# Gavinli-lgf/belief-planning

Hardware: AMD Instinct MI355X
Metric: branch-MPC solves/sec (whole node), highway N=20 M=3 branches, batch 4096 egos (higher is better)
Workload: dtype f64; 1 GPU; highway BranchMPC_CVaR closed loop, N=20, NB=1, m=3 (T=64, U=61), 4096 egos per GPU; batch_per_gpu=4096, global_batch=4096, world_size=1, parallelism=ego-sharded dp1, loop=per step: k_env + solve launches

## Files before the change

### __graft_entry__.py

```python
import os
import sys

REPO = os.path.dirname(os.path.abspath(__file__))
PKG = os.path.join(REPO, "belief-planning_amd")
for _p in (REPO, PKG, os.path.join(REPO, "tests")):
    if _p not in sys.path:
        sys.path.insert(0, _p)


def build() -> None:
    from bmpc import _lib
    _lib.build(force=True, verbose=True)
    _lib.load()
    _lib.build_variant("rec0", ["-DBMPC_ITER_RECORD=0"])
    import hostsim_lib
    hostsim_lib.build()
    import bmpc.plan
    import MPC_branch
    import highway_branch_dyn
    print("build ok:", _lib.SO_PATH)


def smoke() -> None:
    import numpy as np
    from bmpc import plan
    from bmpc.scenarios import highway_desc, highway_policy_rows, seeded_batch
    from oracle.ecos_ipm import ecos_solve
    from oracle.model import HighwayModel, highway_policies
    from oracle.tree import CVaRController
# ... 36 lines not shown
```

### belief-planning_amd/csrc/bmpc_core.h

```cpp
#pragma once

#include <stddef.h>
#include <stdint.h>

#include "bmpc.h"

#ifndef BMPC_PHASE_NOCSR
#define BMPC_PHASE_NOCSR 1
#endif
#if BMPC_PHASE_NOCSR && defined(__HIP_DEVICE_COMPILE__)
#define BMPC_FN_CALLS __attribute__((not_tail_called))
#else
#define BMPC_FN_CALLS
#endif
#ifndef BMPC_ITER_RECORD
#define BMPC_ITER_RECORD 1
#endif
#define BMPC_ITER_LDS 32
#if defined(__HIPCC__)
#include <hip/hip_runtime.h>
#define BMPC_HD __host__ __device__ __forceinline__
#if defined(BMPC_INLINE_ALL)
#define BMPC_FN __host__ __device__ __forceinline__
#else
#define BMPC_FN __host__ __device__ __attribute__((noinline)) BMPC_FN_CALLS
#endif
#else
#define BMPC_HD inline
#define BMPC_FN inline
#endif

// ... 428 lines not shown
```

### belief-planning_amd/csrc/bmpc_ipm.h

```cpp
#pragma once

#include <type_traits>

#include "bmpc_tree.h"
#include "bmpc_wave.h"

#ifndef BMPC_EQUIL
#define BMPC_EQUIL 1
#endif
#ifndef BMPC_EQUIL_ITERS
#define BMPC_EQUIL_ITERS 3
#endif
#ifndef BMPC_TS_POST_RB_MIN
#define BMPC_TS_POST_RB_MIN 8
#endif
#ifndef BMPC_TS_POST_RB
#define BMPC_TS_POST_RB 4
#endif
#ifndef BMPC_PAIR_REFINE
#define BMPC_PAIR_REFINE 1
#endif
#ifndef BMPC_BLK_WAVE_SUBST
#define BMPC_BLK_WAVE_SUBST 1
#endif
// ... 537 lines not shown
  BMPC_TOC(C.ws, *C.L, PROF_G_CONE, t_gcone);
  ex.sync();
}
template <class X, int NX, int NU, int WM>
BMPC_FN_APPLY_G void apply_G_call(const X ex, const Ctx Cin, const gdouble* zv, gdouble* out, const gdouble* r3h,
                                  gdouble* tr) {
  apply_G_body<X, NX, NU, WM>(ex, Cin, zv, out, r3h, tr);
}
template <class X, int NX, int NU, int WM>
BMPC_HD void apply_G(const X ex, const Ctx& C, const gdouble* zv, gdouble* out, const gdouble* r3h, gdouble* tr) {
  if constexpr (inline_g<X>::value) apply_G_body<X, NX, NU, WM>(ex, C, zv, out, r3h, tr);
  else apply_G_call<X, NX, NU, WM>(ex, C, zv, out, r3h, tr);
}

template <class X, int NX, int NU>
BMPC_FN_APPLY_GT void apply_GT(const X ex, const Ctx Cin, const gdouble* r, gdouble* out, const gdouble* add = nullptr) {
  const Ctx C = Cin.uniform();
  add = uniform_ptr(add);
  const double sa = add ? 1.0 : 0.0;
  const gdouble* ad = add ? add : r;
  double qx[NX];
  ctx_qx<NX>(C, qx);
  CPlan& P = *C.P;
  BMPC_PROF(C.ws, *C.L, PROF_APPLYGT);
  const auto t = topo_view(P, ex);
  const int Nc = P.Nc;
  const gdouble* boost = C.at(C.L->boost);
  const gdouble* dh = C.at(C.L->dh);
  const double Qs = P.desc.Qslack[1];
  for (int k = ex.lane; k < P.T; k += ex.nlanes) {
    double ax[NX], cx[NX], os[BMPC_MAX_FX + 1];
#pragma unroll
    for (int j = 0; j < NX; ++j) ax[j] = 0.0, cx[j] = 0.0;
    const bool term = t.x_u[k] < 0;
    double fS = 0.0;
// ... 12 lines not shown
    } else if (k == 0) {
      const int kr = P.ncones - 1;
      const int off = t.cone_off[kr], q = t.cone_q[kr];
      fS = Qs * (r[off] - r[off + q - 1]) * ebeta<X>(boost, P.ncones, kr);
    }
    double dhk[NX];
#pragma unroll
    for (int j = 0; j < NX; ++j) dhk[j] = dh[k * NX + j];
    for (int c = 0; c < Nc; ++c) {
      const double rv = r[P.rFx + k * Nc + c];
      if (!term)
#pragma unroll
        for (int j = 0; j < NX; ++j) ax[j] += (c == 0 ? -dhk[j] : fxv(P, ex, c - 1, j)) * rv;
      os[c] = -rv - r[P.rPos + k * Nc + c] + fS;
    }
    for (int c = 0; c < Nc; ++c) out[P.oS + k * Nc + c] = os[c] + sa * ad[P.oS + k * Nc + c];
#pragma unroll
    for (int j = 0; j < NX; ++j) out[P.oX + k * NX + j] = (kc >= 0 ? ax[j] + cx[j] : ax[j]) + sa * ad[P.oX + k * NX + j];
  }
  for (int u = ex.lane; u < P.U; u += ex.nlanes) {
    double au[NU];
#pragma unroll
    for (int j = 0; j < NU; ++j) au[j] = 0.0;
    for (int rr = 0; rr < P.nFu; ++rr) {
      const double rv = r[P.rFu + u * P.nFu + rr];
#pragma unroll
      for (int j = 0; j < NU; ++j) au[j] += P.desc.Fu[rr * NU + j] * rv;
    }
    const int kc = t.u_cone[u];
    if (kc >= 0) {
      const int off = t.cone_off[kc];
      const int c = t.cone_c[kc];
      const int base = c >= 0 ? 1 + P.N * NX + (u - t.br_ndu[c]) * NU : 1;
#pragma unroll
      for (int s2 = 0; s2 < NU; ++s2) {
        double v = 0.0;
#pragma unroll
        for (int rr = 0; rr < NU; ++rr) v += -2.0 * P.Wu[rr * NU + s2] * r[off + base + rr];
        au[s2] += v;
      }
    }
#pragma unroll
    for (int j = 0; j < NU; ++j) out[P.oU + u * NU + j] = au[j] + sa * ad[P.oU + u * NU + j];
  }
  for (int i = ex.lane; i < P.ng; i += ex.nlanes) {
    double v = 0.0;
    const int gi = i == P.ng - 1 ? P.oJ : P.oRho + i;
    if (gi < P.oSig) v = -r[P.rRisk + (gi - P.oRho)];
    else if (gi >= P.oMup && gi < P.oS) v = -r[P.rRisk + P.bdim + (gi - P.oMup)];
    for (int k = 0; k < P.ncones; ++k) {
      const int off = t.cone_off[k], q = t.cone_q[k], c = t.cone_c[k];
      double w = 0.0;
      if (c >= 0) {
        const int b = t.cone_b[k], ii = t.cone_i[k];
        if (gi == P.oSig + b) w += 1.0;
        if (gi == P.oMup + b + ii) w += 1.0;
        if (gi == P.oMum + b + ii) w -= 1.0;
        if (t.br_child0[c] >= 0 && gi == P.oRho + c) w += 1.0;
      } else {
        if (gi == P.oJ) w -= 1.0;
        if (gi == P.oRho) w += 1.0;
      }
      if (w != 0.0) v += w * (r[off] - r[off + q - 1]) * ebeta<X>(boost, P.ncones, k);
    }
    out[gi] = v + sa * ad[gi];
  }
  ex.sync();
}

template <class X, int NX, int NU>
BMPC_HD void apply_A(const X ex, const Ctx& C, const gdouble* zv, gdouble* out) {
  CPlan& P = *C.P;
  const auto t = topo_view(P, ex);
  const gdouble* Ad = C.at(C.L->Ad);
  const gdouble* Bd = C.at(C.L->Bd);
  struct V4 { double v[NX]; };
  lane_batch<2>(ex, 0, P.T, [&](int k) {
    const int su = t.x_srcu[k], sx = t.x_srcx[k];
    V4 o;
#pragma unroll
    for (int r = 0; r < NX; ++r) o.v[r] = zv[P.oX + k * NX + r];
    if (su >= 0) {
      double xs[NX], us[NU];
// ... 408 lines not shown
#pragma unroll
    for (int uu = 0; uu < UC; ++uu) {
      const int i = G.gl + uu * G.cg;
      if (i < q) out1[off + i] = y[uu];
    }
    cone_W_regs<UC>(ex, G, a, y, cone_row0<UC>(ex, G, y), sc, v);
#pragma unroll
    for (int uu = 0; uu < UC; ++uu) {
      const int i = G.gl + uu * G.cg;
      if (i < q) out2[off + i] = v[uu];
    }
  }
  ex.sync();
}

template <class X>
BMPC_FN_FUSED LpSteps affine_dirs(const X ex, const Ctx Cin, const gdouble* z2, const gdouble* z1, double t,
                                  const gdouble* lam, gdouble* rb, gdouble* ds) {
  const Ctx C = Cin.uniform();
  z2 = uniform_ptr(z2), z1 = uniform_ptr(z1), lam = uniform_ptr(lam), rb = uniform_ptr(rb), ds = uniform_ptr(ds);
  CPlan& P = *C.P;
  LpSteps m{1e300, 1e300};
  if (!cone_regs(ex, P)) {
    gdouble* dz = C.at(C.L->dz);
    lane_batch<8>(ex, 0, P.nrows, [&](int i) { return z2[i] + t * z1[i]; }, [&](int i, double v) { dz[i] = v; });
    ex.sync();
    apply_W(ex, C, 0, dz, rb);
    lane_batch<8>(ex, 0, P.nrows, [&](int i) { return -lam[i] - rb[i]; }, [&](int i, double v) { ds[i] = v; });
    ex.sync();
    return BMPC_IPM_LEAN_PASSES ? lp_steps(ex, P, lam, ds, rb) : m;
// ... 104 lines not shown
        rb[off + i] = y[uu];
        ds[off + i] = d[uu];
      }
    }
    cone_W_regs<UC>(ex, G, a, d, cone_row0<UC>(ex, G, d), sc, v);
#pragma unroll
    for (int uu = 0; uu < UC; ++uu) {
      const int i = G.gl + uu * G.cg;
      if (i < q) rc[off + i] = v[uu];
    }
  }
  ex.sync();
  return m;
}

template <class X>
BMPC_FN_FUSED void combined_rhs(const X ex, const Ctx Cin, const gdouble* lam, gdouble* ds, gdouble* rb,
                                const gdouble* rz, double smu, double eta1) {
  const Ctx C = Cin.uniform();
  lam = uniform_ptr(lam), ds = uniform_ptr(ds), rb = uniform_ptr(rb), rz = uniform_ptr(rz);
  CPlan& P = *C.P;
  if (!cone_regs(ex, P)) {
    gdouble* ra = C.at(C.L->ra);
    gdouble* rc = C.at(C.L->rc);
    jprod(ex, C, lam, lam, ra);
    jprod(ex, C, ds, rb, rc);
    lane_batch<8>(ex, 0, P.nrows, [&](int i) {
      const double v = -ra[i] - rc[i];
      return i < P.nlp ? v + smu : v;
    }, [&](int i, double v) { ra[i] = v; });
    ex.sync();
    for (int k = ex.lane; k < P.ncones; k += ex.nlanes) ra[topo_view(P, ex).cone_off[k]] += smu;
    ex.sync();
    jdiv(ex, C, lam, ra, ds);
    apply_W(ex, C, 0, ds, rb, -1.0, rz, eta1);
    return;
  }
  BMPC_PROF(C.ws, *C.L, PROF_APPLYW);
  constexpr int UC = X::kConeRegRows;
  const gdouble* dl = C.at(C.L->dl);
  struct Two { double a, b; };
  lane_batch<8>(ex, 0, P.nlp, [&](int i) {
    const double l = lam[i];
    const double xi = (-(l * l) - ds[i] * rb[i] + smu) / l;
    return Two{xi, -(dl[i] * xi) + eta1 * rz[i]};
  }, [&](int i, Two v) { ds[i] = v.a; rb[i] = v.b; });
  const gdouble* vn = C.at(C.L->vnt);
  const gdouble* eta = C.at(C.L->eta);
  BMPC_CONE_ROUNDS(ex, P, G) {
    BMPC_CONE_K(P, G, k, off, q);
    double l[UC], bw[UC], r[UC], rzv[UC];
    double pll = 0.0, pdr = 0.0;
#pragma unroll
    for (int uu = 0; uu < UC; ++uu) {
      const int i = G.gl + uu * G.cg;
      const int ic = off + (i < q ? i : 0);
      const double m = i < q ? 1.0 : 0.0;
      const double lv = lam[ic], dv = ds[ic], bv = rb[ic];
      rzv[uu] = rz[ic];
      l[uu] = m * lv;
      bw[uu] = m * bv;
// ... 24 lines not shown
      const int i = G.gl + uu * G.cg;
      if (i >= 1 && i != kidx) pss += l[uu] * l[uu];
    }
    const double ss = ex.gsum(pss, G.cg), lr = ex.gsum(plr, G.cg);
    const double rho = q > 0 ? cone_res_parts(l0, gm, ss) : 1.0;
    const double x0 = q > 0 ? (l0 * r0 - lr) / rho : 0.0;
    double a[UC];
    cone_a_regs<UC, X>(G, vn, false, off, q, a);
#pragma unroll
    for (int uu = 0; uu < UC; ++uu) {
      const int i = G.gl + uu * G.cg;
      r[uu] = i >= q ? 0.0 : i == 0 ? x0 : (r[uu] - x0 * l[uu]) / l0;
    }
    const double sc = -(k >= 0 ? eta[k] : 1.0);
    cone_W_regs<UC>(ex, G, a, r, x0, sc, l);
#pragma unroll
    for (int uu = 0; uu < UC; ++uu) {
      const int i = G.gl + uu * G.cg;
      if (i < q) {
        ds[off + i] = r[uu];
        rb[off + i] = l[uu] + eta1 * rzv[uu];
      }
    }
  }
  ex.sync();
}

BMPC_HD int branch_count(CPlan& P, int dep) {
  int c = 1;
  for (int i = 0; i < dep; ++i) c *= P.m;
  return c;
}
BMPC_HD int branch_start(CPlan& P, int dep) {
  int s = 0, c = 1;
  for (int i = 0; i < dep; ++i) s += c, c *= P.m;
  return s;
}

template <int NX, int NU>
BMPC_HD bool riccati_step(const double (&Hx)[NX][NX], const double (&Hu)[NU][NU], const double (&A)[NX][NX],
// ... 459 lines not shown
    kfv[m] = v;
  }
#pragma unroll
  for (int q = 0; q < RX; ++q) {
    double v = qx[q];
#pragma unroll
    for (int j = 0; j < NX; ++j) v += Acol[q][j] * gfull[j];
#pragma unroll
    for (int m = 0; m < NU; ++m) v += Kcol[q][m] * qu[m];
    l[q] = v;
  }
}

template <class X, int NX, int NU, bool RB = false>
BMPC_FN_TREE_SOLVE void tree_solve(const X ex, const Ctx Cin, int nr, const gdouble* r0, size_t rs, const gdouble* e0,
                        size_t es, gdouble* o0, size_t os, gdouble* n0, size_t ns, int ncw = 0) {
  const Ctx C = Cin.uniform();
  r0 = uniform_ptr(r0);
  e0 = uniform_ptr(e0);
  o0 = uniform_ptr(o0);
  n0 = uniform_ptr(n0);
  constexpr int W = X::kTaskLanes;
  constexpr int RX = (NX + W - 1) / W;
  constexpr int NCM = BMPC_MAX_FX + 1;
  (void)NCM;
  CPlan& P = *C.P;
  CLayout& L = *C.L;
  BMPC_PROF(C.ws, L, PROF_TREESOLVE);
  BMPC_COUNT(C.ws, L, PROF_NTREE);
  const auto t = topo_view(P, ex);
  const int Nc = P.Nc;
  gdouble* ws = C.ws;
// ... 19 lines not shown
      s0[c] = sdv[kc * 2];
      s1[c] = sdv[kc * 2 + 1];
    }
    const double on = t.x_u[k] >= 0 ? 1.0 : 0.0;
    double v = -rr[P.oX + k * NX + i] + dh[k * NX + i] * (on * s1[0] * rS[0] / s0[0]);
#pragma unroll
    for (int c = 1; c < NCM; ++c)
      if (c < Nc) v -= fxv(P, ex, c - 1, i) * (on * s1[c] * rS[c] / s0[c]);
    return v;
  };
  const bool pre = ex.uniform(P.nscr >= P.T * Nc);
  gdouble* q0_ = ws + L.qx0;
  if (pre) {
    BMPC_TIC(t_pre);
    ldouble* av = ex.lds + P.lds_scr;
    for (int ri = 0; ri < nr; ++ri) {
      const gdouble* rr = r0 + ri * rs;
      gdouble* q0 = q0_ + ri * lstr;
      int s0 = 0, l0 = P.T, s1 = 0, l1 = 0, s2 = 0, l2 = 0, s3 = 0, l3 = 0;
      if (ri < ncw) {
        int c = t.cone_c[ri] < 0 ? 0 : t.cone_c[ri];
        int st[4] = {0, 0, 0, 0}, ln[4] = {0, 0, 0, 0};
        bool deeper = true;
#pragma unroll
        for (int q = 0; q < 4; ++q) {
          if (deeper) {
            st[q] = t.br_ndx[c];
            ln[q] = t.br_len[c] + (t.br_child0[c] < 0 ? 1 : 0);
            if (c == 0) deeper = false;
            else c = (c - 1) / P.m;
          }
// ... 621 lines not shown
BMPC_HD auto coup_mem(const X& ex, gdouble* ws, CLayout& L, CPlan& P, int off) {
  if constexpr (X::kCoupLds) return ex.lds + off;
  else return ws + L.coup + (off - P.lds_M);
}
template <class X>
BMPC_HD auto coup_vec(const X& ex, int off) { return ex.lds + off; }


BMPC_HD int gvar(CPlan& P, int i) { return i == P.ng - 1 ? P.oJ : P.oRho + i; }

#if BMPC_THIN_CALLERS
template <class X, int NX, int NU>
BMPC_FN bool kkt_coupling_lu(const X ex, const Ctx Cin);
#endif
template <class X, int NX, int NU>
BMPC_FN bool kkt_coupling(const X ex, const Ctx Cin, int extra) {
  const Ctx C = Cin.uniform();
  CPlan& P = *C.P;
  CLayout& L = *C.L;
  BMPC_PROF(C.ws, L, PROF_COUPLING);
  gdouble* ws = C.ws;
  const int nc = P.ncones;
  BMPC_TIC(t_cts);
  if (ex.uniform(nc + extra >= BMPC_TS_POST_RB_MIN))
    tree_solve<X, NX, NU, true>(ex, C, nc + extra, ws + L.gk, P.nv, ws + L.zeros, P.neq, ws + L.colk, P.nv,
                                ws + L.colnu, P.neq, nc);
  else
    tree_solve<X, NX, NU>(ex, C, nc + extra, ws + L.gk, P.nv, ws + L.zeros, P.neq, ws + L.colk, P.nv, ws + L.colnu,
                          P.neq, nc);
  BMPC_TOC(C.ws, L, PROF_CTS, t_cts);
#if BMPC_THIN_CALLERS
  return kkt_coupling_lu<X, NX, NU>(ex, C);
}
template <class X, int NX, int NU>
BMPC_FN bool kkt_coupling_lu(const X ex, const Ctx Cin) {
  const Ctx C = Cin.uniform();
  CPlan& P = *C.P;
  CLayout& L = *C.L;
  gdouble* ws = C.ws;
  const int nc = P.ncones;
#endif
  BMPC_TIC(t_cdot);
  const int ng = P.ng, nb = P.bdim, ns = P.nsm;
  auto* M = coup_mem(ex, ws, L, P, P.lds_M);
// ... 356 lines not shown
  CLayout& L = *C.L;
  BMPC_PROF(C.ws, L, PROF_KKT);
  gdouble* ws = C.ws;
  gdouble* r3h = ws + L.k_t3;
  apply_Winv2(ex, C, r3, r3h, ws + L.k_r0);
  BMPC_COUNT(ws, L, PROF_NSOLVE);
  const bool fin = ex.uniform(nitref == 0);
  kkt_solve_once<X, NX, NU>(ex, C, r1, r2, r3h, dx, dy, dz, true, fin);
  if (fin) return;
  kkt_refine<X, NX, NU>(ex, C, r1, r2, r3h, dx, dy, dz, nitref);
}

#if BMPC_THIN_CALLERS
template <class X, int NX, int NU>
BMPC_FN void kkt_solve_front(const X ex, const Ctx Cin, const gdouble* r1, const gdouble* r2, const gdouble* r3,
                             gdouble* dx, gdouble* dy) {
  const Ctx C = Cin.uniform();
  r1 = uniform_ptr(r1), r2 = uniform_ptr(r2), r3 = uniform_ptr(r3), dx = uniform_ptr(dx), dy = uniform_ptr(dy);
  CLayout& L = *C.L;
  BMPC_PROF(C.ws, L, PROF_KKT);
  gdouble* ws = C.ws;
  gdouble* tz = ws + L.k_nv0;
  apply_Winv2(ex, C, r3, ws + L.k_t3, ws + L.k_r0);
  BMPC_COUNT(ws, L, PROF_NSOLVE);
  apply_GT<X, NX, NU>(ex, C, ws + L.k_r0, tz, r1);
  tree_solve<X, NX, NU>(ex, C, 1, tz, 0, r2, 0, dx, 0, dy, 0);
}
template <class X, int NX, int NU>
BMPC_FN void kkt_solve_back(const X ex, const Ctx Cin, const gdouble* r2, gdouble* dx, gdouble* dy, gdouble* dz,
                            bool fin) {
  const Ctx C = Cin.uniform();
  fin = ex.uniform(fin);
  CLayout& L = *C.L;
  BMPC_PROF(C.ws, L, PROF_KKT);
  kkt_back<X, NX, NU, false>(ex, C, C.ws + L.k_nv0, r2, C.ws + L.k_t3, dx, dy, dz, fin);
}
template <class X, int NX, int NU>
BMPC_FN void kkt_refine_call(const X ex, const Ctx Cin, const gdouble* r1, const gdouble* r2, gdouble* dx, gdouble* dy,
                             gdouble* dz, int nitref) {
  const Ctx C = Cin.uniform();
  r1 = uniform_ptr(r1), r2 = uniform_ptr(r2), dx = uniform_ptr(dx), dy = uniform_ptr(dy), dz = uniform_ptr(dz);
  BMPC_PROF(C.ws, *C.L, PROF_KKT);
  kkt_refine<X, NX, NU>(ex, C, r1, r2, C.ws + C.L->k_t3, dx, dy, dz, nitref);
}
template <class X, int NX, int NU>
BMPC_HD void kkt_solve_flat(const X ex, const Ctx& C, const gdouble* r1, const gdouble* r2, const gdouble* r3,
                            gdouble* dx, gdouble* dy, gdouble* dz, int nitref) {
  kkt_solve_front<X, NX, NU>(ex, C, r1, r2, r3, dx, dy);
  const bool fin = ex.uniform(nitref == 0);
  kkt_solve_back<X, NX, NU>(ex, C, r2, dx, dy, dz, fin);
  if (!fin) kkt_refine_call<X, NX, NU>(ex, C, r1, r2, dx, dy, dz, nitref);
}
#else
template <class X, int NX, int NU>
BMPC_HD void kkt_solve_flat(const X ex, const Ctx& C, const gdouble* r1, const gdouble* r2, const gdouble* r3,
                            gdouble* dx, gdouble* dy, gdouble* dz, int nitref) {
  kkt_solve<X, NX, NU>(ex, C, r1, r2, r3, dx, dy, dz, nitref);
}
#endif

template <class X, int NX, int NU>
BMPC_HD void kkt_refine(const X ex, const Ctx& C, const gdouble* r1, const gdouble* r2, const gdouble* r3h,
                        gdouble* dx, gdouble* dy, gdouble* dz, int nitref) {
  CPlan& P = *C.P;
  CLayout& L = *C.L;
  gdouble* ws = C.ws;
  gdouble* e1 = ws + L.k_e1;
  gdouble* e2 = ws + L.k_e2;
  gdouble* e3 = ws + L.k_e3;
  gdouble* cx = ws + L.k_cx;
  gdouble* cy = ws + L.k_cy;
// ... 226 lines not shown
}

#if BMPC_FLAT_PAIR
template <class X, int NX, int NU>
BMPC_FN void kkt_pair_rhs(const X ex, const Ctx Cin, const gdouble* r1c, const gdouble* r1a, const gdouble* r3a) {
  const Ctx C = Cin.uniform();
  r1c = uniform_ptr(r1c), r1a = uniform_ptr(r1a), r3a = uniform_ptr(r3a);
  CPlan& P = *C.P;
  CLayout& L = *C.L;
  BMPC_PROF(C.ws, L, PROF_KKT);
  gdouble* ws = C.ws;
  const size_t nv = P.nv, nc = P.ncones;
  gdouble* tzc = ws + L.gk + nc * nv;
  gdouble* tza = tzc + nv;
  gdouble* tr = ws + L.k_r0;
  apply_Winv2(ex, C, ws + L.hvec, ws + L.k_t3, tr);
  apply_GT<X, NX, NU>(ex, C, tr, tzc, r1c);
  apply_Winv2(ex, C, r3a, ws + L.k_t3b, tr);
  apply_GT<X, NX, NU>(ex, C, tr, tza, r1a);
  BMPC_COUNT(ws, L, PROF_NSOLVE);
  BMPC_COUNT(ws, L, PROF_NSOLVE);
}
template <class X, int NX, int NU>
BMPC_FN void kkt_pair_back(const X ex, const Ctx Cin, bool fin) {
  const Ctx C = Cin.uniform();
  fin = ex.uniform(fin);
  CPlan& P = *C.P;
  CLayout& L = *C.L;
  BMPC_PROF(C.ws, L, PROF_KKT);
  gdouble* ws = C.ws;
  const size_t nv = P.nv, nc = P.ncones;
  const gdouble* tzc = ws + L.gk + nc * nv;
  const gdouble* tza = tzc + nv;
#if BMPC_PAIR_BACK
// ... 552 lines not shown
      return res;
    }
    const int nref = ex.uniform(score < BMPC_REFSCORE2) ? BMPC_NITREF2 : ex.uniform(score < BMPC_REFSCORE) ? BMPC_NITREF : 0;
    bool ok = ex.uniform(compute_scaling(ex, C, ws + LL().s, ws + LL().z));
    if (ok) ok = ex.uniform(kkt_factor<X, NX, NU>(ex, C, false));
    if (ok) {
      gdouble* ej = BMPC_IPM_LEAN_PASSES ? ws + LL().ej : ws + LL().ta;
#if !BMPC_IPM_LEAN_PASSES
      {
        const gdouble* rx = ws + LL().rx;
        gdouble* tA2 = ws + LL().ta2;
        lane_batch<16>(ex, 0, nv, [&](int i) { return i == P.oJ ? -1.0 : 0.0; }, [&](int i, double v) { ej[i] = v; });
        lane_batch<16>(ex, 0, nv, [&](int i) { return -rx[i]; }, [&](int i, double v) { tA2[i] = v; });
      }
#endif
      apply_W(ex, C, 0, ws + LL().lam, ws + LL().rb, 1.0, ws + LL().rz, 1.0);
#if BMPC_FLAT_PAIR
      kkt_pair_rhs<X, NX, NU>(ex, C, ej, ws + LL().ta2, ws + LL().rb);
      ok = ex.uniform(kkt_coupling<X, NX, NU>(ex, C, 2));
      if (ok) {
        kkt_pair_back<X, NX, NU>(ex, C, nref == 0);
        if (nref > 0) {
#if BMPC_PAIR_REFINE
          kkt_refine_pair<X, NX, NU>(ex, C, ej, ws + LL().bvec, ws + LL().k_t3, ws + LL().x1, ws + LL().y1, ws + LL().z1, ws + LL().ta2,
                                     ws + LL().ry, ws + LL().k_t3b, ws + LL().x2, ws + LL().y2, ws + LL().z2, nref);
#else
          kkt_refine<X, NX, NU>(ex, C, ej, ws + LL().bvec, ws + LL().k_t3, ws + LL().x1, ws + LL().y1, ws + LL().z1, nref);
          kkt_refine<X, NX, NU>(ex, C, ws + LL().ta2, ws + LL().ry, ws + LL().k_t3b, ws + LL().x2, ws + LL().y2, ws + LL().z2, nref);
#endif
        }
      }
#else
      ok = ex.uniform(kkt_solve_pair<X, NX, NU>(ex, C, ej, ws + LL().ta2, ws + LL().rb, nref));
#endif
// ... 18 lines not shown
      const LpSteps lpa = affine_dirs(ex, C, ws + LL().z2, ws + LL().z1, R.ld(IT_DTAU_A), ws + LL().lam, ws + LL().rb, ws + LL().ds);
      double a_aff = max_step2<X, BMPC_IPM_LEAN_PASSES != 0>(ex, C, ws + LL().lam, ws + LL().ds, ws + LL().rb, lpa.a1, lpa.a2);
      {
        const double tau = R.ld(IT_TAU), kap = R.ld(IT_KAP);
        const double dtau_a = R.ld(IT_DTAU_A), dkap_a = R.ld(IT_DKAP_A);
        if (dtau_a < 0.0) a_aff = fmin(a_aff, -tau / dtau_a);
        if (dkap_a < 0.0) a_aff = fmin(a_aff, -kap / dkap_a);
        a_aff = fmax(0.0, fmin(a_aff, 0.999));
        double sigma = (1.0 - a_aff) * (1.0 - a_aff) * (1.0 - a_aff);
        sigma = fmin(1.0, fmax(1e-4, sigma));
        const double eta1 = 1.0 - sigma;
        const double smu = sigma * R.ld(IT_MU);
        R.st(IT_SIGMA, sigma);
        R.st(IT_ETA1, eta1);
        R.st(IT_SMU, smu);
        combined_rhs(ex, C, ws + LL().lam, ws + LL().ds, ws + LL().rb, ws + LL().rz, smu, eta1);
      }
      {
        const gdouble* rx = ws + LL().rx;
        const gdouble* ry = ws + LL().ry;
        gdouble* tA = ws + LL().ta;
        gdouble* ya = ws + LL().ya;
        const double eta1 = R.ld(IT_ETA1);
        lane_batch<16>(ex, 0, nv, [&](int i) { return -eta1 * rx[i]; }, [&](int i, double v) { tA[i] = v; });
        lane_batch(ex, 0, neq, [&](int i) { return eta1 * ry[i]; }, [&](int i, double v) { ya[i] = v; });
        ex.sync();
      }
      kkt_solve_flat<X, NX, NU>(ex, C, ws + LL().ta, ws + LL().ya, ws + LL().rb, ws + LL().x2, ws + LL().y2, ws + LL().z2, nref);
      {
        const double d2 = dot2(ex, ws + LL().bvec, ws + LL().y2, neq, ws + LL().hvec, ws + LL().z2, nr);
        const double tau = R.ld(IT_TAU);
        const double dk_c = -R.ld(IT_KT) - R.ld(IT_DTAU_A) * R.ld(IT_DKAP_A) + R.ld(IT_SMU);
        const double dtau = (R.ld(IT_ETA1) * R.ld(IT_RT) + dk_c / tau + ws[LL().x2 + P.oJ] + d2) / R.ld(IT_DEN);
        R.st(IT_DTAU, dtau);
        R.st(IT_DKAP, (dk_c - R.ld(IT_KAP) * dtau) / tau);
      }
      double nonfinite = 0.0;
#if !BMPC_IPM_LEAN_PASSES
      {
        const gdouble* x1 = ws + LL().x1;
        const gdouble* y1 = ws + LL().y1;
        gdouble* x2 = ws + LL().x2;
        gdouble* y2 = ws + LL().y2;
// ... 291 lines not shown
      ex.sync();
      res.exit_flag = code;
      res.iters = it;
      res.pcost = pcost;
      return res;
    }
    bool ok = ex.uniform(compute_scaling(ex, C, s, z));
    if (ok) ok = ex.uniform(kkt_factor<X, NX, NU>(ex, C, false));
    double alpha = 0.0, dtau = 0.0, dkap = 0.0;
    const int nref = score < BMPC_REFSCORE2 ? BMPC_NITREF2 : score < BMPC_REFSCORE ? BMPC_NITREF : 0;
    if (ok) {
#if !BMPC_IPM_LEAN_PASSES
      lane_batch<16>(ex, 0, nv, [&](int i) { return i == P.oJ ? -1.0 : 0.0; }, [&](int i, double v) { ej[i] = v; });
      lane_batch<16>(ex, 0, nv, [&](int i) { return -rx[i]; }, [&](int i, double v) { tA2[i] = v; });
#endif
      apply_W(ex, C, 0, lam, rb, 1.0, rz, 1.0);
#if BMPC_FLAT_PAIR
      kkt_pair_rhs<X, NX, NU>(ex, C, ej, tA2, rb);
      ok = ex.uniform(kkt_coupling<X, NX, NU>(ex, C, 2));
      if (ok) {
        kkt_pair_back<X, NX, NU>(ex, C, nref == 0);
        if (nref > 0) {
#if BMPC_PAIR_REFINE
          kkt_refine_pair<X, NX, NU>(ex, C, ej, bv, ws + L.k_t3, x1, y1, z1, tA2, ry, ws + L.k_t3b, x2, y2, z2, nref);
#else
          kkt_refine<X, NX, NU>(ex, C, ej, bv, ws + L.k_t3, x1, y1, z1, nref);
          kkt_refine<X, NX, NU>(ex, C, tA2, ry, ws + L.k_t3b, x2, y2, z2, nref);
#endif
        }
      }
#else
      ok = ex.uniform(kkt_solve_pair<X, NX, NU>(ex, C, ej, tA2, rb, nref));
#endif
    }
// ... 4 lines not shown
#else
      const double by1 = dot2(ex, bv, y1, neq, hv, z1, nr), by2 = dot2(ex, bv, y2, neq, hv, z2, nr);
#endif
      const double den = kap / tau - (x1[P.oJ] + by1);
      const double dk_aff = -kap * tau;
      const double dtau_a = (rt + dk_aff / tau + x2[P.oJ] + by2) / den;
      const LpSteps lpa = affine_dirs(ex, C, z2, z1, dtau_a, lam, rb, ds);
      const double dkap_a = (dk_aff - kap * dtau_a) / tau;
      double a_aff = max_step2<X, BMPC_IPM_LEAN_PASSES != 0>(ex, C, lam, ds, rb, lpa.a1, lpa.a2);
      if (dtau_a < 0.0) a_aff = fmin(a_aff, -tau / dtau_a);
      if (dkap_a < 0.0) a_aff = fmin(a_aff, -kap / dkap_a);
      a_aff = fmax(0.0, fmin(a_aff, 0.999));
      double sigma = (1.0 - a_aff) * (1.0 - a_aff) * (1.0 - a_aff);
      sigma = fmin(1.0, fmax(1e-4, sigma));
      const double eta1 = 1.0 - sigma;
      combined_rhs(ex, C, lam, ds, rb, rz, sigma * mu, eta1);
      lane_batch<16>(ex, 0, nv, [&](int i) { return -eta1 * rx[i]; }, [&](int i, double v) { tA[i] = v; });
      lane_batch(ex, 0, neq, [&](int i) { return eta1 * ry[i]; }, [&](int i, double v) { ya[i] = v; });
      ex.sync();
      kkt_solve_flat<X, NX, NU>(ex, C, tA, ya, rb, x2, y2, z2, nref);
      const double dk_c = -kap * tau - dtau_a * dkap_a + sigma * mu;
      dtau = (eta1 * rt + dk_c / tau + x2[P.oJ] + dot2(ex, bv, y2, neq, hv, z2, nr)) / den;
      double nonfinite = 0.0;
#if !BMPC_IPM_LEAN_PASSES
      lane_batch<8>(ex, 0, nv, [&](int i) { return x2[i] + (dtau * x1[i]); }, [&](int i, double v) {
        x2[i] = v;
        if (!isfinite(v)) nonfinite = 1.0;
      });
      lane_batch(ex, 0, neq, [&](int i) { return y2[i] + (dtau * y1[i]); }, [&](int i, double v) { y2[i] = v; });
      ex.sync();
#endif
      const LpSteps lpc = combined_dirs(ex, C, z2, z1, dtau, ds, rb, rc);
      dkap = (dk_c - kap * dtau) / tau;
      double a = max_step2<X, BMPC_IPM_LEAN_PASSES != 0>(ex, C, lam, ds, rb, lpc.a1, lpc.a2);
      if (dtau < 0.0) a = fmin(a, -tau / dtau);
// ... 71 lines not shown
```

Measured before the change: 84240 solves/s.

## Fuse W/Winv scaling into RHS kernels and fold eta1 scaling into apply_GT

Adds register-resident fused kernels. The affine right-hand side now computes W*lam+rz followed by the double W-inverse in one pass. The combined RHS writes the W-inverse-applied vectors directly. apply_GT gains a scale argument, so the -eta1*rx vector no longer has to be materialised separately. An optional q0 precomputation path is added but disabled by default. The aim is to cut separate global-memory passes and syncs in each IPM iteration, at the cost of more code paths and more register pressure.

```diff
diff --git a/__graft_entry__.py b/__graft_entry__.py
--- a/__graft_entry__.py
+++ b/__graft_entry__.py
@@ -13,6 +13,7 @@
     _lib.build(force=True, verbose=True)
     _lib.load()
     _lib.build_variant("rec0", ["-DBMPC_ITER_RECORD=0"])
+    _lib.build_variant("rhs0", ["-DBMPC_RHS_AFF_REGS=0", "-DBMPC_RHS_CMB_REGS=0", "-DBMPC_GT_Q0=0", "-DBMPC_GT_SCALED_ADD=0"])
     import hostsim_lib
     hostsim_lib.build()
     import bmpc.plan
diff --git a/belief-planning_amd/csrc/bmpc_core.h b/belief-planning_amd/csrc/bmpc_core.h
--- a/belief-planning_amd/csrc/bmpc_core.h
+++ b/belief-planning_amd/csrc/bmpc_core.h
@@ -15,6 +15,18 @@
 #endif
 #ifndef BMPC_ITER_RECORD
 #define BMPC_ITER_RECORD 1
+#endif
+#ifndef BMPC_RHS_AFF_REGS
+#define BMPC_RHS_AFF_REGS 1
+#endif
+#ifndef BMPC_RHS_CMB_REGS
+#define BMPC_RHS_CMB_REGS 1
+#endif
+#ifndef BMPC_GT_Q0
+#define BMPC_GT_Q0 0
+#endif
+#ifndef BMPC_GT_SCALED_ADD
+#define BMPC_GT_SCALED_ADD 1
 #endif
 #define BMPC_ITER_LDS 32
 #if defined(__HIPCC__)
diff --git a/belief-planning_amd/csrc/bmpc_ipm.h b/belief-planning_amd/csrc/bmpc_ipm.h
--- a/belief-planning_amd/csrc/bmpc_ipm.h
+++ b/belief-planning_amd/csrc/bmpc_ipm.h
@@ -575,11 +575,24 @@
 }
 
 template <class X, int NX, int NU>
-BMPC_FN_APPLY_GT void apply_GT(const X ex, const Ctx Cin, const gdouble* r, gdouble* out, const gdouble* add = nullptr) {
+BMPC_FN_APPLY_GT void apply_GT(const X ex, const Ctx Cin, const gdouble* r, gdouble* out, const gdouble* add = nullptr,
+                               double asc = 1.0, gdouble* q0 = nullptr) {
   const Ctx C = Cin.uniform();
   add = uniform_ptr(add);
   const double sa = add ? 1.0 : 0.0;
+#if BMPC_GT_Q0
+  q0 = uniform_ptr(q0);
+  const bool toq0 = ex.uniform(q0 != nullptr);
+  const gdouble* sdv = C.at(C.L->sd);
+#endif
+#if BMPC_GT_SCALED_ADD
+  const gdouble* adp = add ? add : r;
+  auto ad = [&](int i) { return asc * adp[i]; };
+#define BMPC_GT_AD(i) ad(i)
+#else
   const gdouble* ad = add ? add : r;
+#define BMPC_GT_AD(i) ad[i]
+#endif
   double qx[NX];
   ctx_qx<NX>(C, qx);
   CPlan& P = *C.P;
@@ -622,9 +635,34 @@
         for (int j = 0; j < NX; ++j) ax[j] += (c == 0 ? -dhk[j] : fxv(P, ex, c - 1, j)) * rv;
       os[c] = -rv - r[P.rPos + k * Nc + c] + fS;
     }
-    for (int c = 0; c < Nc; ++c) out[P.oS + k * Nc + c] = os[c] + sa * ad[P.oS + k * Nc + c];
-#pragma unroll
-    for (int j = 0; j < NX; ++j) out[P.oX + k * NX + j] = (kc >= 0 ? ax[j] + cx[j] : ax[j]) + sa * ad[P.oX + k * NX + j];
+#if BMPC_GT_Q0
+    if (toq0) {
+      constexpr int NCM = BMPC_MAX_FX + 1;
+      const double on = term ? 0.0 : 1.0;
+      double av[NCM], rX[NX];
+#pragma unroll
+      for (int c = 0; c < NCM; ++c) {
+        const int it = k * Nc + (c < Nc ? c : 0);
+        const double rS = os[c < Nc ? c : 0] + sa * BMPC_GT_AD(P.oS + it);
+        av[c] = on * sdv[it * 2 + 1] * rS / sdv[it * 2];
+        if (c < Nc) out[P.oS + it] = rS;
+      }
+#pragma unroll
+      for (int j = 0; j < NX; ++j) rX[j] = (kc >= 0 ? ax[j] + cx[j] : ax[j]) + sa * BMPC_GT_AD(P.oX + k * NX + j);
+#pragma unroll
+      for (int j = 0; j < NX; ++j) {
+        double v = -rX[j] + dhk[j] * av[0];
+#pragma unroll
+        for (int c = 1; c < NCM; ++c)
+          if (c < Nc) v -= fxv(P, ex, c - 1, j) * av[c];
+        q0[k * NX + j] = v;
+      }
+      continue;
+    }
+#endif
+    for (int c = 0; c < Nc; ++c) out[P.oS + k * Nc + c] = os[c] + sa * BMPC_GT_AD(P.oS + k * Nc + c);
+#pragma unroll
+    for (int j = 0; j < NX; ++j) out[P.oX + k * NX + j] = (kc >= 0 ? ax[j] + cx[j] : ax[j]) + sa * BMPC_GT_AD(P.oX + k * NX + j);
   }
   for (int u = ex.lane; u < P.U; u += ex.nlanes) {
     double au[NU];
@@ -649,7 +687,7 @@
       }
     }
 #pragma unroll
-    for (int j = 0; j < NU; ++j) out[P.oU + u * NU + j] = au[j] + sa * ad[P.oU + u * NU + j];
+    for (int j = 0; j < NU; ++j) out[P.oU + u * NU + j] = au[j] + sa * BMPC_GT_AD(P.oU + u * NU + j);
   }
   for (int i = ex.lane; i < P.ng; i += ex.nlanes) {
     double v = 0.0;
@@ -671,10 +709,11 @@
       }
       if (w != 0.0) v += w * (r[off] - r[off + q - 1]) * ebeta<X>(boost, P.ncones, k);
     }
-    out[gi] = v + sa * ad[gi];
+    out[gi] = v + sa * BMPC_GT_AD(gi);
   }
   ex.sync();
 }
+#undef BMPC_GT_AD
 
 template <class X, int NX, int NU>
 BMPC_HD void apply_A(const X ex, const Ctx& C, const gdouble* zv, gdouble* out) {
@@ -1113,6 +1152,88 @@
   ex.sync();
 }
 
+template <class X, class = void>
+struct rhs_regs_exec { static constexpr bool value = true; };
+template <class X>
+struct rhs_regs_exec<X, decltype((void)X::kIterRecord)> { static constexpr bool value = X::kIterRecord; };
+
+template <class X>
+BMPC_HD bool gt_q0(const X&, CPlan& P) {
+  return BMPC_GT_Q0 && BMPC_THIN_CALLERS && BMPC_FLAT_PAIR && rhs_regs_exec<X>::value && P.nscr >= P.T * P.Nc;
+}
+
+#if BMPC_RHS_AFF_REGS
+template <class X>
+BMPC_HD bool rhs_aff_regs(const X& ex, CPlan& P) {
+  return rhs_regs_exec<X>::value && cone_regs(ex, P) && P.maxq <= 8 * exec_cgrp(ex, P.cgrp, P.ncones);
+}
+template <class X>
+BMPC_FN_FUSED void apply_Winv2_aff(const X ex, const Ctx Cin, const gdouble* lam, const gdouble* rz, gdouble* out1,
+                                   gdouble* out2) {
+  const Ctx C = Cin.uniform();
+  lam = uniform_ptr(lam), rz = uniform_ptr(rz), out1 = uniform_ptr(out1), out2 = uniform_ptr(out2);
+  CPlan& P = *C.P;
+  BMPC_PROF(C.ws, *C.L, PROF_APPLYW);
+  constexpr int UC = X::kConeRegRows;
+  const double sw = 1.0, sa = 1.0;
+  const gdouble* dl = C.at(C.L->dl);
+  const gdouble* dli = C.at(C.L->dli);
+  struct Two { double a, b; };
+  lane_batch<8>(ex, 0, P.nlp, [&](int i) {
+    const double in = sw * (dl[i] * lam[i]) + sa * rz[i];
+    const double w = dli[i];
+    const double a = w * in;
+    return Two{a, w * a};
+  }, [&](int i, Two v) { out1[i] = v.a; out2[i] = v.b; });
+  const gdouble* vn = C.at(C.L->vnt);
+  const gdouble* eta = C.at(C.L->eta);
+  BMPC_CONE_ROUNDS(ex, P, G) {
+    BMPC_CONE_K(P, G, k, off, q);
+    double a[UC], v[UC], y[UC], aw[UC];
+    const double e = k >= 0 ? eta[k] : 1.0;
+    const double in0 = q > 0 ? lam[off] : 0.0;
+    double part = 0.0;
+#pragma unroll
+    for (int uu = 0; uu < UC; ++uu) {
+      const int i = G.gl + uu * G.cg;
+      const int ic = off + (i < q ? i : 0);
+      const double m = i < q ? 1.0 : 0.0;
+      aw[uu] = m * vn[ic];
+      y[uu] = m * lam[ic];
+      part += aw[uu] * y[uu];
+    }
+    const double dot = ex.gsum(part, G.cg);
+#pragma unroll
+    for (int uu = 0; uu < UC; ++uu) {
+      const int i = G.gl + uu * G.cg;
+      const double adv = (i < q ? 1.0 : 0.0) * rz[off + (i < q ? i : 0)];
+      const double w = 2.0 * aw[uu] * dot - (i == 0 ? in0 : -y[uu]);
+#if defined(__HIP_DEVICE_COMPILE__)
+      const double t = __builtin_fma(sw * e, w, sa * adv);
+#else
+      const double t = (sw * e) * w + sa * adv;
+#endif
+      v[uu] = i < q ? t : 0.0;
+    }
+    cone_a_regs<UC, X>(G, vn, true, off, q, a);
+    const double sc = 1.0 / e;
+    cone_W_regs<UC>(ex, G, a, v, cone_row0<UC>(ex, G, v), sc, y);
+#pragma unroll
+    for (int uu = 0; uu < UC; ++uu) {
+      const int i = G.gl + uu * G.cg;
+      if (i < q) out1[off + i] = y[uu];
+    }
+    cone_W_regs<UC>(ex, G, a, y, cone_row0<UC>(ex, G, y), sc, v);
+#pragma unroll
+    for (int uu = 0; uu < UC; ++uu) {
+      const int i = G.gl + uu * G.cg;
+      if (i < q) out2[off + i] = v[uu];
+    }
+  }
+  ex.sync();
+}
+#endif
+
 template <class X>
 BMPC_FN_FUSED LpSteps affine_dirs(const X ex, const Ctx Cin, const gdouble* z2, const gdouble* z1, double t,
                                   const gdouble* lam, gdouble* rb, gdouble* ds) {
@@ -1247,11 +1368,12 @@
   return m;
 }
 
-template <class X>
-BMPC_FN_FUSED void combined_rhs(const X ex, const Ctx Cin, const gdouble* lam, gdouble* ds, gdouble* rb,
-                                const gdouble* rz, double smu, double eta1) {
+template <class X, bool WINV>
+BMPC_HD void combined_rhs_body(const X ex, const Ctx Cin, const gdouble* lam, gdouble* ds, gdouble* rb,
+                               const gdouble* rz, double smu, double eta1, gdouble* t3, gdouble* t0) {
   const Ctx C = Cin.uniform();
   lam = uniform_ptr(lam), ds = uniform_ptr(ds), rb = uniform_ptr(rb), rz = uniform_ptr(rz);
+  if constexpr (WINV) t3 = uniform_ptr(t3), t0 = uniform_ptr(t0);
   CPlan& P = *C.P;
   if (!cone_regs(ex, P)) {
     gdouble* ra = C.at(C.L->ra);
@@ -1273,11 +1395,24 @@
   constexpr int UC = X::kConeRegRows;
   const gdouble* dl = C.at(C.L->dl);
   struct Two { double a, b; };
+  if constexpr (WINV) {
+    const gdouble* dli = C.at(C.L->dli);
+    struct Three { double x, a, b; };
+    lane_batch<8>(ex, 0, P.nlp, [&](int i) {
+      const double l = lam[i];
+      const double xi = (-(l * l) - ds[i] * rb[i] + smu) / l;
+      const double in = -(dl[i] * xi) + eta1 * rz[i];
+      const double w = dli[i];
+      const double a = w * in;
+      return Three{xi, a, w * a};
+    }, [&](int i, Three v) { ds[i] = v.x; t3[i] = v.a; t0[i] = v.b; });
+  } else {
   lane_batch<8>(ex, 0, P.nlp, [&](int i) {
     const double l = lam[i];
     const double xi = (-(l * l) - ds[i] * rb[i] + smu) / l;
     return Two{xi, -(dl[i] * xi) + eta1 * rz[i]};
   }, [&](int i, Two v) { ds[i] = v.a; rb[i] = v.b; });
+  }
   const gdouble* vn = C.at(C.L->vnt);
   const gdouble* eta = C.at(C.L->eta);
   BMPC_CONE_ROUNDS(ex, P, G) {
@@ -1332,6 +1467,29 @@
     }
     const double sc = -(k >= 0 ? eta[k] : 1.0);
     cone_W_regs<UC>(ex, G, a, r, x0, sc, l);
+    if constexpr (WINV) {
+#pragma unroll
+      for (int uu = 0; uu < UC; ++uu) {
+        const int i = G.gl + uu * G.cg;
+        const double t = l[uu] + eta1 * rzv[uu];
+        if (i < q) ds[off + i] = r[uu];
+        l[uu] = i < q ? t : 0.0;
+        a[uu] = (i > 0 && i < q) ? -a[uu] : a[uu];
+      }
+      const double sci = 1.0 / (k >= 0 ? eta[k] : 1.0);
+      cone_W_regs<UC>(ex, G, a, l, cone_row0<UC>(ex, G, l), sci, r);
+#pragma unroll
+      for (int uu = 0; uu < UC; ++uu) {
+        const int i = G.gl + uu * G.cg;
+        if (i < q) t3[off + i] = r[uu];
+      }
+      cone_W_regs<UC>(ex, G, a, r, cone_row0<UC>(ex, G, r), sci, l);
+#pragma unroll
+      for (int uu = 0; uu < UC; ++uu) {
+        const int i = G.gl + uu * G.cg;
+        if (i < q) t0[off + i] = l[uu];
+      }
+    } else {
 #pragma unroll
     for (int uu = 0; uu < UC; ++uu) {
       const int i = G.gl + uu * G.cg;
@@ -1340,8 +1498,25 @@
         rb[off + i] = l[uu] + eta1 * rzv[uu];
       }
     }
+    }
   }
   ex.sync();
+}
+template <class X>
+BMPC_FN_FUSED void combined_rhs(const X ex, const Ctx Cin, const gdouble* lam, gdouble* ds, gdouble* rb,
+                                const gdouble* rz, double smu, double eta1) {
+  combined_rhs_body<X, false>(ex, Cin, lam, ds, rb, rz, smu, eta1, nullptr, nullptr);
+}
+#if BMPC_RHS_CMB_REGS
+template <class X>
+BMPC_FN_FUSED void combined_rhs_winv(const X ex, const Ctx Cin, const gdouble* lam, gdouble* ds, const gdouble* rb,
+                                     const gdouble* rz, double smu, double eta1, gdouble* t3, gdouble* r0) {
+  combined_rhs_body<X, true>(ex, Cin, lam, ds, const_cast<gdouble*>(rb), rz, smu, eta1, t3, r0);
+}
+#endif
+template <class X>
+BMPC_HD bool rhs_cmb_regs(const X& ex, CPlan& P) {
+  return BMPC_RHS_CMB_REGS && BMPC_THIN_CALLERS && rhs_regs_exec<X>::value && cone_regs(ex, P);
 }
 
 BMPC_HD int branch_count(CPlan& P, int dep) {
@@ -1831,8 +2006,9 @@
 
 template <class X, int NX, int NU, bool RB = false>
 BMPC_FN_TREE_SOLVE void tree_solve(const X ex, const Ctx Cin, int nr, const gdouble* r0, size_t rs, const gdouble* e0,
-                        size_t es, gdouble* o0, size_t os, gdouble* n0, size_t ns, int ncw = 0) {
+                        size_t es, gdouble* o0, size_t os, gdouble* n0, size_t ns, int ncw = 0, int nq0 = 0) {
   const Ctx C = Cin.uniform();
+  nq0 = BMPC_GT_Q0 ? ex.uniform(nq0 != 0) ? nq0 : 0 : 0;
   r0 = uniform_ptr(r0);
   e0 = uniform_ptr(e0);
   o0 = uniform_ptr(o0);
@@ -1882,7 +2058,7 @@
   if (pre) {
     BMPC_TIC(t_pre);
     ldouble* av = ex.lds + P.lds_scr;
-    for (int ri = 0; ri < nr; ++ri) {
+    for (int ri = 0; ri < nr - nq0; ++ri) {
       const gdouble* rr = r0 + ri * rs;
       gdouble* q0 = q0_ + ri * lstr;
       int s0 = 0, l0 = P.T, s1 = 0, l1 = 0, s2 = 0, l2 = 0, s3 = 0, l3 = 0;
@@ -2534,7 +2710,7 @@
 BMPC_FN bool kkt_coupling_lu(const X ex, const Ctx Cin);
 #endif
 template <class X, int NX, int NU>
-BMPC_FN bool kkt_coupling(const X ex, const Ctx Cin, int extra) {
+BMPC_FN bool kkt_coupling(const X ex, const Ctx Cin, int extra, int nq0 = 0) {
   const Ctx C = Cin.uniform();
   CPlan& P = *C.P;
   CLayout& L = *C.L;
@@ -2544,10 +2720,10 @@
   BMPC_TIC(t_cts);
   if (ex.uniform(nc + extra >= BMPC_TS_POST_RB_MIN))
     tree_solve<X, NX, NU, true>(ex, C, nc + extra, ws + L.gk, P.nv, ws + L.zeros, P.neq, ws + L.colk, P.nv,
-                                ws + L.colnu, P.neq, nc);
+                                ws + L.colnu, P.neq, nc, nq0);
   else
     tree_solve<X, NX, NU>(ex, C, nc + extra, ws + L.gk, P.nv, ws + L.zeros, P.neq, ws + L.colk, P.nv, ws + L.colnu,
-                          P.neq, nc);
+                          P.neq, nc, nq0);
   BMPC_TOC(C.ws, L, PROF_CTS, t_cts);
 #if BMPC_THIN_CALLERS
   return kkt_coupling_lu<X, NX, NU>(ex, C);
@@ -2934,17 +3110,21 @@
 #if BMPC_THIN_CALLERS
 template <class X, int NX, int NU>
 BMPC_FN void kkt_solve_front(const X ex, const Ctx Cin, const gdouble* r1, const gdouble* r2, const gdouble* r3,
-                             gdouble* dx, gdouble* dy) {
+                             gdouble* dx, gdouble* dy, double r1s = 1.0, bool q0 = false) {
   const Ctx C = Cin.uniform();
   r1 = uniform_ptr(r1), r2 = uniform_ptr(r2), r3 = uniform_ptr(r3), dx = uniform_ptr(dx), dy = uniform_ptr(dy);
   CLayout& L = *C.L;
   BMPC_PROF(C.ws, L, PROF_KKT);
   gdouble* ws = C.ws;
   gdouble* tz = ws + L.k_nv0;
+#if BMPC_RHS_CMB_REGS
+  if (!ex.uniform(r3 == nullptr))
+#endif
   apply_Winv2(ex, C, r3, ws + L.k_t3, ws + L.k_r0);
   BMPC_COUNT(ws, L, PROF_NSOLVE);
-  apply_GT<X, NX, NU>(ex, C, ws + L.k_r0, tz, r1);
-  tree_solve<X, NX, NU>(ex, C, 1, tz, 0, r2, 0, dx, 0, dy, 0);
+  q0 = ex.uniform(q0);
+  apply_GT<X, NX, NU>(ex, C, ws + L.k_r0, tz, r1, r1s, q0 ? ws + L.qx0 : nullptr);
+  tree_solve<X, NX, NU>(ex, C, 1, tz, 0, r2, 0, dx, 0, dy, 0, 0, q0 ? 1 : 0);
 }
 template <class X, int NX, int NU>
 BMPC_FN void kkt_solve_back(const X ex, const Ctx Cin, const gdouble* r2, gdouble* dx, gdouble* dy, gdouble* dz,
@@ -2965,8 +3145,8 @@
 }
 template <class X, int NX, int NU>
 BMPC_HD void kkt_solve_flat(const X ex, const Ctx& C, const gdouble* r1, const gdouble* r2, const gdouble* r3,
-                            gdouble* dx, gdouble* dy, gdouble* dz, int nitref) {
-  kkt_solve_front<X, NX, NU>(ex, C, r1, r2, r3, dx, dy);
+                            gdouble* dx, gdouble* dy, gdouble* dz, int nitref, double r1s = 1.0, bool q0 = false) {
+  kkt_solve_front<X, NX, NU>(ex, C, r1, r2, r3, dx, dy, r1s, q0);
   const bool fin = ex.uniform(nitref == 0);
   kkt_solve_back<X, NX, NU>(ex, C, r2, dx, dy, dz, fin);
   if (!fin) kkt_refine_call<X, NX, NU>(ex, C, r1, r2, dx, dy, dz, nitref);
@@ -2974,7 +3154,7 @@
 #else
 template <class X, int NX, int NU>
 BMPC_HD void kkt_solve_flat(const X ex, const Ctx& C, const gdouble* r1, const gdouble* r2, const gdouble* r3,
-                            gdouble* dx, gdouble* dy, gdouble* dz, int nitref) {
+                            gdouble* dx, gdouble* dy, gdouble* dz, int nitref, double = 1.0, bool = false) {
   kkt_solve<X, NX, NU>(ex, C, r1, r2, r3, dx, dy, dz, nitref);
 }
 #endif
@@ -3231,10 +3411,15 @@
   gdouble* tzc = ws + L.gk + nc * nv;
   gdouble* tza = tzc + nv;
   gdouble* tr = ws + L.k_r0;
+  gdouble* q0 = ex.uniform(gt_q0(ex, P)) ? ws + L.qx0 + nc * ((size_t)P.T * NX) : nullptr;
   apply_Winv2(ex, C, ws + L.hvec, ws + L.k_t3, tr);
-  apply_GT<X, NX, NU>(ex, C, tr, tzc, r1c);
+  apply_GT<X, NX, NU>(ex, C, tr, tzc, r1c, 1.0, q0);
+#if BMPC_RHS_AFF_REGS
+  if (ex.uniform(rhs_aff_regs(ex, P))) apply_Winv2_aff(ex, C, ws + L.lam, ws + L.rz, ws + L.k_t3b, tr);
+  else
+#endif
   apply_Winv2(ex, C, r3a, ws + L.k_t3b, tr);
-  apply_GT<X, NX, NU>(ex, C, tr, tza, r1a);
+  apply_GT<X, NX, NU>(ex, C, tr, tza, r1a, 1.0, q0 ? q0 + (size_t)P.T * NX : nullptr);
   BMPC_COUNT(ws, L, PROF_NSOLVE);
   BMPC_COUNT(ws, L, PROF_NSOLVE);
 }
@@ -3817,10 +4002,13 @@
         lane_batch<16>(ex, 0, nv, [&](int i) { return -rx[i]; }, [&](int i, double v) { tA2[i] = v; });
       }
 #endif
+#if BMPC_RHS_AFF_REGS && BMPC_FLAT_PAIR
+      if (!ex.uniform(rhs_aff_regs(ex, P)))
+#endif
       apply_W(ex, C, 0, ws + LL().lam, ws + LL().rb, 1.0, ws + LL().rz, 1.0);
 #if BMPC_FLAT_PAIR
       kkt_pair_rhs<X, NX, NU>(ex, C, ej, ws + LL().ta2, ws + LL().rb);
-      ok = ex.uniform(kkt_coupling<X, NX, NU>(ex, C, 2));
+      ok = ex.uniform(kkt_coupling<X, NX, NU>(ex, C, 2, ex.uniform(gt_q0(ex, P)) ? 2 : 0));
       if (ok) {
         kkt_pair_back<X, NX, NU>(ex, C, nref == 0);
         if (nref > 0) {
@@ -3869,19 +4057,35 @@
         R.st(IT_SIGMA, sigma);
         R.st(IT_ETA1, eta1);
         R.st(IT_SMU, smu);
+#if BMPC_RHS_CMB_REGS
+        if (ex.uniform(rhs_cmb_regs(ex, P)))
+          combined_rhs_winv(ex, C, ws + LL().lam, ws + LL().ds, ws + LL().rb, ws + LL().rz, smu, eta1, ws + LL().k_t3, ws + LL().k_r0);
+        else
+#endif
         combined_rhs(ex, C, ws + LL().lam, ws + LL().ds, ws + LL().rb, ws + LL().rz, smu, eta1);
       }
+      const bool r1_scaled = ex.uniform(BMPC_GT_SCALED_ADD && BMPC_THIN_CALLERS && rhs_regs_exec<X>::value && nref == 0);
       {
         const gdouble* rx = ws + LL().rx;
         const gdouble* ry = ws + LL().ry;
         gdouble* tA = ws + LL().ta;
         gdouble* ya = ws + LL().ya;
         const double eta1 = R.ld(IT_ETA1);
-        lane_batch<16>(ex, 0, nv, [&](int i) { return -eta1 * rx[i]; }, [&](int i, double v) { tA[i] = v; });
+        if (!r1_scaled) lane_batch<16>(ex, 0, nv, [&](int i) { return -eta1 * rx[i]; }, [&](int i, double v) { tA[i] = v; });
         lane_batch(ex, 0, neq, [&](int i) { return eta1 * ry[i]; }, [&](int i, double v) { ya[i] = v; });
         ex.sync();
       }
-      kkt_solve_flat<X, NX, NU>(ex, C, ws + LL().ta, ws + LL().ya, ws + LL().rb, ws + LL().x2, ws + LL().y2, ws + LL().z2, nref);
+      {
+        const gdouble* r3 = ex.uniform(rhs_cmb_regs(ex, P)) ? nullptr : ws + LL().rb;
+#if BMPC_GT_SCALED_ADD
+        if (r1_scaled)
+          kkt_solve_flat<X, NX, NU>(ex, C, ws + LL().rx, ws + LL().ya, r3, ws + LL().x2, ws + LL().y2, ws + LL().z2, nref, -R.ld(IT_ETA1),
+                                    ex.uniform(gt_q0(ex, P)));
+        else
+#endif
+        kkt_solve_flat<X, NX, NU>(ex, C, ws + LL().ta, ws + LL().ya, r3, ws + LL().x2, ws + LL().y2, ws + LL().z2, nref, 1.0,
+                                  ex.uniform(gt_q0(ex, P)));
+      }
       {
         const double d2 = dot2(ex, ws + LL().bvec, ws + LL().y2, neq, ws + LL().hvec, ws + LL().z2, nr);
         const double tau = R.ld(IT_TAU);
@@ -4203,10 +4407,13 @@
       lane_batch<16>(ex, 0, nv, [&](int i) { return i == P.oJ ? -1.0 : 0.0; }, [&](int i, double v) { ej[i] = v; });
       lane_batch<16>(ex, 0, nv, [&](int i) { return -rx[i]; }, [&](int i, double v) { tA2[i] = v; });
 #endif
+#if BMPC_RHS_AFF_REGS && BMPC_FLAT_PAIR
+      if (!ex.uniform(rhs_aff_regs(ex, P)))
+#endif
       apply_W(ex, C, 0, lam, rb, 1.0, rz, 1.0);
 #if BMPC_FLAT_PAIR
       kkt_pair_rhs<X, NX, NU>(ex, C, ej, tA2, rb);
-      ok = ex.uniform(kkt_coupling<X, NX, NU>(ex, C, 2));
+      ok = ex.uniform(kkt_coupling<X, NX, NU>(ex, C, 2, ex.uniform(gt_q0(ex, P)) ? 2 : 0));
       if (ok) {
         kkt_pair_back<X, NX, NU>(ex, C, nref == 0);
         if (nref > 0) {
@@ -4241,11 +4448,23 @@
       double sigma = (1.0 - a_aff) * (1.0 - a_aff) * (1.0 - a_aff);
       sigma = fmin(1.0, fmax(1e-4, sigma));
       const double eta1 = 1.0 - sigma;
+#if BMPC_RHS_CMB_REGS
+      if (ex.uniform(rhs_cmb_regs(ex, P))) combined_rhs_winv(ex, C, lam, ds, rb, rz, sigma * mu, eta1, ws + L.k_t3, ws + L.k_r0);
+      else
+#endif
       combined_rhs(ex, C, lam, ds, rb, rz, sigma * mu, eta1);
-      lane_batch<16>(ex, 0, nv, [&](int i) { return -eta1 * rx[i]; }, [&](int i, double v) { tA[i] = v; });
+      const bool r1_scaled = ex.uniform(BMPC_GT_SCALED_ADD && BMPC_THIN_CALLERS && rhs_regs_exec<X>::value && nref == 0);
+      if (!r1_scaled) lane_batch<16>(ex, 0, nv, [&](int i) { return -eta1 * rx[i]; }, [&](int i, double v) { tA[i] = v; });
       lane_batch(ex, 0, neq, [&](int i) { return eta1 * ry[i]; }, [&](int i, double v) { ya[i] = v; });
       ex.sync();
-      kkt_solve_flat<X, NX, NU>(ex, C, tA, ya, rb, x2, y2, z2, nref);
+      {
+        const gdouble* r3 = ex.uniform(rhs_cmb_regs(ex, P)) ? nullptr : rb;
+#if BMPC_GT_SCALED_ADD
+        if (r1_scaled) kkt_solve_flat<X, NX, NU>(ex, C, rx, ya, r3, x2, y2, z2, nref, -eta1, ex.uniform(gt_q0(ex, P)));
+        else
+#endif
+        kkt_solve_flat<X, NX, NU>(ex, C, tA, ya, r3, x2, y2, z2, nref, 1.0, ex.uniform(gt_q0(ex, P)));
+      }
       const double dk_c = -kap * tau - dtau_a * dkap_a + sigma * mu;
       dtau = (eta1 * rt + dk_c / tau + x2[P.oJ] + dot2(ex, bv, y2, neq, hv, z2, nr)) / den;
       double nonfinite = 0.0;
```

Result: faster. 85480 solves/s, median of 6 (+1.5%).
